# codelion/adaptive-classifier

Hardware: AMD Instinct MI355X
Metric: predict() queries/sec + kNN GB/s vs HBM roofline, 768-d (higher is better)
Workload: dtype f32

## Files before the change

adaptive-classifier_amd/adaptive_classifier/_native.py:

```python
import ctypes
import os
import subprocess

import torch

_HERE = os.path.dirname(os.path.abspath(__file__))
_LIB_PATH = os.environ.get("AC_LIBACAMD_PATH") or os.path.join(_HERE, "libacamd.so")
_CSRC = os.path.join(os.path.dirname(_HERE), "csrc")
_lib = None

c_void_p, c_int, c_int64, c_size_t, c_float, c_uint64 = (
    ctypes.c_void_p, ctypes.c_int, ctypes.c_int64, ctypes.c_size_t, ctypes.c_float, ctypes.c_uint64)


class NativeError(RuntimeError):
    pass


AC_GEMM_F32, AC_GEMM_BF16X3, AC_GEMM_F16X2 = 0, 1, 2
AC_BERT_LAYERED = 1
AC_BERT_PATH_PACKED, AC_BERT_PATH_PADDED, AC_BERT_PATH_PADDED_MASK = 0, 1, 2


def build(force=False):
# ... 31 lines not shown
        "attn_norm_g", "attn_norm_b", "wqkv", "wqkv_b", "wo", "wo_b", "mlp_norm_g", "mlp_norm_b",
        "wi", "wi_b", "wo2", "wo2_b", "zero_bias", "wqkv3", "wo3", "wi3", "wo23")] + [("wi_interleaved32", c_int)]


class ac_wordpiece_vocab(ctypes.Structure):
    _fields_ = [("keys", c_void_p), ("offs", c_void_p), ("ids", c_void_p), ("lens", c_void_p), ("blob", c_void_p),
                ("slots", c_int), ("max_piece_bytes", c_int), ("unk_id", c_int), ("cls_id", c_int), ("sep_id", c_int),
                ("pad_id", c_int), ("lower_case", c_int)]


class ac_bert_weights(ctypes.Structure):
    _fields_ = [(n, c_void_p) for n in (
        "word_emb", "pos_emb", "type_emb", "emb_ln_g", "emb_ln_b",
        "qkv_w", "qkv_b", "ao_w", "ao_b", "ln1_g", "ln1_b",
        "ff1_w", "ff1_b", "ff2_w", "ff2_b", "ln2_g", "ln2_b",
        "qkv_w3", "ao_w3", "ff1_w3", "ff2_w3", "qkv_wh", "ao_wh", "ff1_wh", "ff2_wh")]


_SIGNATURES = {
    "ac_last_error": (ctypes.c_char_p, []),
    "ac_version": (c_int, []),
    "ac_device_info": (c_int, [ctypes.POINTER(c_int), ctypes.POINTER(c_int), ctypes.POINTER(c_size_t)]),
    "ac_device_cus": (c_int, [ctypes.POINTER(c_int), ctypes.POINTER(c_int)]),
    "ac_persistent_launches": (c_int, [ctypes.POINTER(c_int64), ctypes.POINTER(c_int64)]),
    "ac_knn_l2_topk_workspace": (c_int, [c_int64, c_int, c_int, c_int, ctypes.POINTER(c_size_t)]),
    "ac_knn_l2_topk": (c_int, [c_void_p, c_int64, c_int64, c_int, c_void_p, c_int, c_int64, c_int, c_int64,
                               c_void_p, c_void_p, c_void_p, c_size_t, c_void_p, c_void_p]),
    "ac_knn_l2_topk_x": (c_int, [c_void_p, c_int64, c_int64, c_int, c_void_p, c_int, c_int64, c_int, c_int64,
                                 c_void_p, c_void_p, c_void_p, c_void_p, c_size_t, c_void_p, c_void_p]),
    "ac_knn_ip_topk_workspace": (c_int, [c_int64, c_int, c_int, c_int, ctypes.POINTER(c_size_t)]),
    "ac_knn_ip_topk": (c_int, [c_void_p, c_int64, c_int64, c_int, c_void_p, c_int, c_int64, c_int, c_int64,
                               c_void_p, c_void_p, c_void_p, c_size_t, c_void_p, c_void_p]),
    "ac_knn_ip_topk_x": (c_int, [c_void_p, c_int64, c_int64, c_int, c_void_p, c_int, c_int64, c_int, c_int64,
                                 c_void_p, c_void_p, c_void_p, c_void_p, c_size_t, c_void_p, c_void_p]),
    "ac_topk_merge_ip_f64": (c_int, [c_void_p, c_void_p, c_int, c_int, c_int, c_void_p, c_void_p, c_void_p]),
    "ac_knn_store_bytes": (c_int, [c_int64, c_int, ctypes.POINTER(c_size_t), ctypes.POINTER(c_size_t)]),
    "ac_knn_prepare_store": (c_int, [c_void_p, c_int64, c_int64, c_int, c_void_p, c_void_p, c_void_p]),
    "ac_knn_update_store": (c_int, [c_void_p, c_int64, c_int64, c_int64, c_int, c_void_p, c_void_p, c_int64, c_int64, c_void_p, c_void_p]),
    "ac_knn_l2_topk_batch_workspace": (c_int, [c_int64, c_int, c_int, c_int, ctypes.POINTER(c_size_t)]),
    "ac_knn_l2_topk_batch": (c_int, [c_void_p, c_int64, c_int64, c_int, c_void_p, c_void_p, c_void_p, c_int, c_int64, c_int,
                                     c_int64, c_void_p, c_void_p, c_void_p, c_void_p, c_size_t, c_void_p, c_void_p]),
    "ac_knn_ip_topk_batch_workspace": (c_int, [c_int64, c_int, c_int, c_int, ctypes.POINTER(c_size_t)]),
    "ac_knn_ip_topk_batch": (c_int, [c_void_p, c_int64, c_int64, c_int, c_void_p, c_void_p, c_void_p, c_int, c_int64, c_int,
                                     c_int64, c_void_p, c_void_p, c_void_p, c_void_p, c_size_t, c_void_p, c_void_p]),
    "ac_knn_range_workspace": (c_int, [c_int64, c_int, c_int, ctypes.POINTER(c_size_t)]),
    "ac_knn_l2_range_count": (c_int, [c_void_p, c_int64, c_int64, c_int, c_void_p, c_int, c_int64, c_void_p, c_void_p,
                                      c_void_p, c_size_t, c_void_p, c_void_p]),
    "ac_knn_l2_range_fill": (c_int, [c_void_p, c_int64, c_int64, c_int, c_void_p, c_int, c_int64, c_int64, c_void_p, c_int64,
                                     c_void_p, c_void_p, c_void_p, c_void_p, c_size_t, c_void_p, c_void_p]),
    "ac_knn_ip_range_count": (c_int, [c_void_p, c_int64, c_int64, c_int, c_void_p, c_int, c_int64, c_void_p, c_void_p,
                                      c_void_p, c_size_t, c_void_p, c_void_p]),
    "ac_knn_ip_range_fill": (c_int, [c_void_p, c_int64, c_int64, c_int, c_void_p, c_int, c_int64, c_int64, c_void_p, c_int64,
                                     c_void_p, c_void_p, c_void_p, c_void_p, c_size_t, c_void_p, c_void_p]),
    "ac_knn_l2_topk_sel": (c_int, [c_void_p, c_int64, c_int64, c_int, c_void_p, c_int, c_int64, c_int, c_int64, c_void_p, c_int64,
                                   c_void_p, c_void_p, c_void_p, c_void_p, c_size_t, c_void_p, c_void_p]),
    "ac_knn_ip_topk_sel": (c_int, [c_void_p, c_int64, c_int64, c_int, c_void_p, c_int, c_int64, c_int, c_int64, c_void_p, c_int64,
                                   c_void_p, c_void_p, c_void_p, c_void_p, c_size_t, c_void_p, c_void_p]),
    "ac_knn_l2_topk_ids": (c_int, [c_void_p, c_int64, c_int64, c_int, c_void_p, c_int64, c_void_p, c_int, c_int64, c_int, c_int64,
                                   c_void_p, c_void_p, c_void_p, c_void_p]),
    "ac_knn_ip_topk_ids": (c_int, [c_void_p, c_int64, c_int64, c_int, c_void_p, c_int64, c_void_p, c_int, c_int64, c_int, c_int64,
                                   c_void_p, c_void_p, c_void_p, c_void_p]),
    "ac_knn_sel_pack": (c_int, [c_void_p, c_int64, c_void_p, c_void_p]),
    "ac_knn_sel_classes": (c_int, [c_void_p, c_int64, c_void_p, c_int, c_void_p, c_void_p]),
    "ac_knn_set_profile_events": (c_int, [c_void_p, c_void_p]),
    "ac_topk_merge": (c_int, [c_void_p, c_void_p, c_int, c_int, c_int, c_void_p, c_void_p, c_void_p]),
    "ac_topk_merge_f64": (c_int, [c_void_p, c_void_p, c_int, c_int, c_int, c_void_p, c_void_p, c_void_p]),
    "ac_rows_to_class": (c_int, [c_void_p, c_int64, c_void_p, c_int64, c_void_p, c_int, c_void_p, c_void_p]),
    "ac_proto_scores": (c_int, [c_void_p, c_void_p, c_int, c_int, c_void_p, c_void_p]),
    "ac_synth_unit_rows": (c_int, [c_void_p, c_int64, c_int64, c_int, c_uint64, c_int64, c_void_p]),
    "ac_linear_f32": (c_int, [c_void_p, c_int64, c_void_p, c_int64, c_void_p, c_void_p, c_int64, c_void_p,
                              c_int64, c_int, c_int, c_int, c_int, c_void_p]),
    "ac_gemm_f32": (c_int, [c_int, c_int, c_int, c_int, c_int, c_float, c_void_p, c_int64, c_void_p, c_int64,
                            c_float, c_void_p, c_int64, c_void_p]),
    "ac_gemm_set_arith": (c_int, [c_int]),
    "ac_gemm_get_arith": (c_int, []),
    "ac_gemm_set_variant": (c_int, [c_int]),
    "ac_gemm_debug_stamps": (c_int, [c_void_p, c_int64]),
    "ac_gemm_set_pipe_table": (c_int, [ctypes.c_char_p]),
    "ac_gemm_set_pipe_table_f16": (c_int, [ctypes.c_char_p]),
    "ac_gemm_set_krot": (c_int, [c_int]),
    "ac_gemm_set_ln_fusion": (c_int, [c_int]),
    "ac_gemm_ln_fusion_launches": (c_int64, []),
    "ac_gemm_qkv_attn_launches": (c_int64, []),
    "ac_set_persistent_kernels": (c_int, [c_int]),
    "ac_clock_stamp": (c_int, [c_void_p, c_void_p]),
    "ac_gemm_occupancy": (c_int, [c_int, c_int, ctypes.POINTER(c_int)]),
    "ac_split_bf16x3": (c_int, [c_void_p, c_int64, c_int64, c_int, c_void_p, c_void_p]),
    "ac_split_f16x2": (c_int, [c_void_p, c_int64, c_int64, c_int, c_int, c_void_p, c_void_p]),
    "ac_linear_f16x2": (c_int, [c_void_p, c_void_p, c_void_p, c_void_p, c_int64, c_void_p, c_int64, c_void_p, c_int, c_int,
                                c_int, c_int, c_void_p]),
    "ac_linear_bf16x3": (c_int, [c_void_p, c_int64, c_void_p, c_void_p, c_int64, c_void_p, c_void_p, c_void_p,
                                 c_int64, c_void_p, c_int64, c_void_p, c_int, c_int, c_int, c_int, c_void_p]),
    "ac_head_param_count": (c_int64, [ctypes.POINTER(ac_head_dims)]),
    "ac_head_workspace": (c_int, [ctypes.POINTER(ac_head_dims), c_int, ctypes.POINTER(c_size_t)]),
    "ac_head_forward": (c_int, [ctypes.POINTER(ac_head_dims), c_void_p, c_void_p, c_int64, c_int, c_void_p,
                                c_void_p, c_size_t, c_void_p]),
    "ac_head_fwd_bwd_ce": (c_int, [ctypes.POINTER(ac_head_dims), c_void_p, c_void_p, c_int64, c_void_p,
                                   c_void_p, c_void_p, c_float, c_int, c_void_p, c_void_p, c_void_p, c_size_t,
                                   c_void_p]),
    "ac_head_fwd_bwd_loss": (c_int, [ctypes.POINTER(ac_head_dims), c_void_p, c_void_p, c_int64, c_void_p, c_void_p,
                                     c_int64, c_int, c_void_p, c_void_p, c_float, c_int, c_void_p, c_void_p, c_void_p,
                                     c_size_t, c_void_p]),
    "ac_strategic_workspace": (c_int, [ctypes.POINTER(ac_head_dims), c_int, c_int, ctypes.POINTER(c_size_t)]),
    "ac_strategic_best_response": (c_int, [ctypes.POINTER(ac_head_dims), c_void_p, c_void_p, c_int64, c_int, c_void_p,
                                           c_void_p, c_int, c_void_p, c_int, c_int, c_void_p, c_void_p, c_float, c_uint64,
                                           c_void_p, c_void_p, c_void_p, c_void_p, c_int64, c_void_p, c_void_p, c_size_t,
                                           c_void_p]),
    "ac_head_fwd_bwd_strategic": (c_int, [ctypes.POINTER(ac_head_dims), c_void_p, c_void_p, c_int64, c_void_p, c_void_p,
                                          c_void_p, c_float, c_int, c_uint64, c_int, c_float, c_void_p, c_void_p, c_void_p,
                                          c_void_p, c_size_t, c_void_p]),
    "ac_sigmoid": (c_int, [c_void_p, c_int64, c_void_p, c_void_p]),
    "ac_head_train_step": (c_int, [ctypes.POINTER(ac_head_dims), c_void_p, c_void_p, c_void_p, c_void_p, c_void_p,
                                   c_int64, c_void_p, c_void_p, c_int64, c_int, c_void_p, c_int, c_float, c_uint64,
                                   c_void_p, c_void_p,
                                   c_float, c_float, c_float, c_float, c_float, c_float, c_float, c_int, c_void_p,
                                   c_void_p, c_void_p, c_size_t, c_void_p]),
    "ac_head_train_epoch": (c_int, [ctypes.POINTER(ac_head_dims), c_void_p, c_void_p, c_void_p, c_void_p, c_void_p,
                                    c_int64, c_void_p, c_void_p, c_int64, c_int, c_void_p, c_int64, c_int, c_float,
                                    c_uint64, c_void_p, c_void_p,
                                    c_float, c_float, c_float, c_float, c_float, c_float, c_float, c_int, c_void_p,
                                    c_void_p, c_void_p, c_size_t, ctypes.POINTER(c_int), c_void_p]),
    "ac_softmax_rows": (c_int, [c_void_p, c_int, c_int, c_void_p, c_void_p]),
    "ac_l2_normalize_rows": (c_int, [c_void_p, c_int64, c_int, c_int, c_void_p, c_int64, c_void_p]),
    "ac_fisher_accumulate": (c_int, [c_void_p, c_float, c_void_p, c_int64, c_void_p]),
    "ac_ewc_loss": (c_int, [c_void_p, c_void_p, c_void_p, c_int64, c_float, c_void_p, c_void_p, c_void_p]),
    "ac_ewc_adamw_step": (c_int, [c_void_p, c_void_p, c_void_p, c_void_p, c_void_p, c_void_p, c_int64, c_float,
                                  c_float, c_float, c_float, c_float, c_float, c_float, c_int, c_void_p,
                                  c_void_p, c_void_p]),
    "ac_memory_add_prune": (c_int, [c_void_p, c_void_p, c_int, c_int, c_void_p]),
    "ac_blend_topk": (c_int, [c_void_p, c_void_p, c_int, c_void_p, c_int, c_void_p, c_void_p, c_int, c_int, c_int,
                              c_void_p, c_void_p, c_void_p, c_void_p]),
    "ac_modernbert_workspace": (c_int, [ctypes.POINTER(ac_modernbert_config), c_int, c_int, ctypes.POINTER(c_size_t)]),
    "ac_modernbert_encode_cls": (c_int, [ctypes.POINTER(ac_modernbert_config), ctypes.POINTER(ac_modernbert_weights),
                                         c_void_p, c_void_p, c_int, c_int, c_void_p, c_int64, c_void_p, c_size_t,
                                         c_void_p]),
    "ac_modernbert_encode_cls_packed": (c_int, [ctypes.POINTER(ac_modernbert_config), ctypes.POINTER(ac_modernbert_weights),
                                                c_void_p, c_int, c_int, c_void_p, c_void_p, c_int, c_int, c_void_p, c_int64,
                                                c_void_p, c_size_t, c_void_p]),
    "ac_wordpiece_hash": (c_uint64, [c_void_p, c_int, c_int]),
    "ac_wordpiece_encode": (c_int, [c_void_p, c_void_p, c_int, ctypes.POINTER(ac_wordpiece_vocab), c_int, c_void_p, c_void_p,
                                    c_void_p, c_void_p]),
    "ac_bert_workspace": (c_int, [ctypes.POINTER(ac_bert_config), c_int, c_int, ctypes.POINTER(c_size_t)]),
    "ac_bert_pack": (c_int, [c_void_p, c_int, c_int, c_void_p, c_void_p, c_void_p, c_void_p]),
    "ac_bert_encode_cls_packed": (c_int, [ctypes.POINTER(ac_bert_config), ctypes.POINTER(ac_bert_weights), c_void_p, c_void_p,
                                          c_int, c_int, c_void_p, c_void_p, c_int, c_int, c_void_p, c_int64, c_void_p, c_size_t,
                                          c_void_p]),
    "ac_bert_unpad_last_wait_ns": (ctypes.c_longlong, []),
    "ac_predict_post": (c_int, [c_void_p, c_void_p, c_int, c_void_p, c_int64, c_void_p, c_int, c_void_p, c_int, c_int, c_void_p, c_void_p,
                                c_int, c_int, c_int, c_void_p, c_size_t, c_void_p, c_void_p]),
    "ac_host_alloc": (c_int, [c_size_t, ctypes.POINTER(c_void_p)]),
    "ac_host_free": (c_int, [c_void_p]),
    "ac_bert_encode_cls_unpad": (c_int, [ctypes.POINTER(ac_bert_config), ctypes.POINTER(ac_bert_weights), c_void_p, c_void_p,
                                         c_void_p, c_int, c_int, c_void_p, c_int64, c_void_p, c_size_t, c_int,
                                         ctypes.POINTER(c_int), ctypes.POINTER(c_int), c_void_p]),
    "ac_bert_encode_cls_opts": (c_int, [ctypes.POINTER(ac_bert_config), ctypes.POINTER(ac_bert_weights), c_void_p,
                                        c_void_p, c_void_p, c_int, c_int, c_void_p, c_int64, c_void_p, c_size_t, c_int,
                                        ctypes.POINTER(c_int), c_void_p]),
    "ac_bert_one_launch_status": (c_int, [ctypes.POINTER(ac_bert_config), c_int, c_int, c_void_p, c_size_t,
                                          ctypes.POINTER(c_int), c_void_p]),
    "ac_bert_ln_fusion_clear": (c_int, [c_void_p, c_size_t, c_void_p]),
    "ac_bert_ln_fusion_status": (c_int, [ctypes.POINTER(ac_bert_config), c_int, c_int, c_void_p, c_size_t,
                                         ctypes.POINTER(c_int), c_void_p]),
    "ac_bert_encode_cls": (c_int, [ctypes.POINTER(ac_bert_config), ctypes.POINTER(ac_bert_weights), c_void_p,
                                   c_void_p, c_void_p, c_int, c_int, c_void_p, c_int64, c_void_p, c_size_t,
                                   c_void_p]),
}
# ... 54 lines not shown
```

adaptive-classifier_amd/csrc/bert.hip:

```cpp
#include "common.h"
#include "attention_core.h"

#include <math.h>
#include <atomic>
#include <chrono>
#include <string.h>

namespace {

typedef float f32x4 __attribute__((ext_vector_type(4)));
constexpr int kMaxVec = 8;

__device__ __forceinline__ float wave_sum(float v) {
#pragma unroll
    for (int o = 1; o < 64; o <<= 1) v += __shfl_xor(v, o);
    return v;
}

template <bool F16 = false>
__device__ __forceinline__ void layernorm_store(f32x4 (&x)[kMaxVec], int H, int lane, const float* g,
                                                const float* b, float eps, float* dst, uint16_t* planes = nullptr,
                                                int64_t rows = 0, int64_t row = 0) {
    const int nv = H >> 2;
    float s = 0.f;
// ... 575 lines not shown
            ac::linear_f16x2_takes(T, H, I);
    return p;
}
void launch_embed(const ac_bert_config& c, const ac_bert_weights* w, const EncodePlan& pn, const int64_t* d_ids, const int64_t* d_type_ids,
                  int rows, int S, float* x, uint16_t* xp, const int32_t* tok_src, const int32_t* t_dev, hipStream_t stream) {
    const int H = c.hidden, tok_blocks = (rows + 3) / 4;
    if (pn.f16)
        hipLaunchKernelGGL(embed_ln_kernel<true>, dim3(tok_blocks), dim3(256), 0, stream, d_ids, d_type_ids, rows, S, H,
                           w->word_emb, w->pos_emb, w->type_emb, w->emb_ln_g, w->emb_ln_b, c.ln_eps, x, xp, tok_src, t_dev);
    else
        hipLaunchKernelGGL(embed_ln_kernel<false>, dim3(tok_blocks), dim3(256), 0, stream, d_ids, d_type_ids, rows, S, H,
                           w->word_emb, w->pos_emb, w->type_emb, w->emb_ln_g, w->emb_ln_b, c.ln_eps, x,
                           pn.pl ? xp : nullptr, tok_src, t_dev);
}
constexpr int kPreCtl = 1, kPreEmbed = 2;
int bert_encode_impl(const ac_bert_config* cfg, const ac_bert_weights* w, const int64_t* d_ids, const int64_t* d_type_ids,
                     const int64_t* d_mask, int b, int S, const int32_t* cu, const int32_t* tok_src, int T, int Smax,
                     float* d_out, int64_t ldo, void* d_ws, size_t ws_bytes, hipStream_t stream, int pre = 0) {
    int rc;
    const ac_bert_config& c = *cfg;
    const BertWs ws = bert_ws(c, b, S);
    AC_REQUIRE(d_ws && ws_bytes >= ws.total, AC_EWORKSPACE, "bert_encode_cls: workspace %zu < %zu", ws_bytes, ws.total);
    char* base = (char*)d_ws;
    float* x = (float*)(base + ws.x);
    float* qkv = (float*)(base + ws.qkv);
    float* ctx = (float*)(base + ws.ctx);
    float* y = (float*)(base + ws.y);
    float* ffn = (float*)(base + ws.ffn);
    const int H = c.hidden, I = c.intermediate;

    uint16_t* xp = (uint16_t*)(base + ws.xp);
    uint16_t* ctxp = (uint16_t*)(base + ws.ctxp);
    uint16_t* ffnp = (uint16_t*)(base + ws.ffnp);
    const EncodePlan pn = encode_plan(c, w, T);
    const bool wplanes = pn.wplanes, pl = pn.pl;
    const bool f16 = pn.f16;
    const bool fuse_ln = pl && c.layers > 1 && ac::pipe_ln_applies(T, H, H) && ac::pipe_ln_applies(T, H, I);
    unsigned* ln_abort = (unsigned*)base;
    if (!(pre & kPreCtl)) {
        hipLaunchKernelGGL(ln_verdict_roll_kernel, dim3(1), dim3(1), 0, stream, ln_abort);
        AC_LAUNCH_CHECK();
    }
    unsigned* ln_count = (unsigned*)(base + ws.lnctl);
    const int ln_panels = ac::pipe_ln_panels(T);
    if (fuse_ln && !(pre & kPreCtl)) AC_HIP_CHECK(hipMemsetAsync(base + ws.lnctl, 0, ws.lnctl_bytes, stream));

    if (!(pre & kPreEmbed)) {
        launch_embed(c, w, pn, d_ids, d_type_ids, T, S, x, xp, tok_src, nullptr, stream);
        AC_LAUNCH_CHECK();
    }
    const int dh = c.hidden / c.heads;
    const float scale = 1.0f / sqrtf((float)dh);
    const int32_t* cu_at = cu;
    const bool fuse_attn = pl && c.layers > 1 && dh == 64 && (cu || !d_mask) && ac::qkv_attn_applies(T, H, c.heads, Smax);
    if (fuse_attn && !cu) {
        int32_t* cuw = (int32_t*)(base + ws.cu);
        hipLaunchKernelGGL(iota_cu_kernel, dim3((b + 256) / 256), dim3(256), 0, stream, cuw, b, S);
        AC_LAUNCH_CHECK();
        cu_at = cuw;
    }
    int32_t* tile_seq = (int32_t*)(base + ws.tile_seq);
    unsigned* attn_xchg = nullptr;
    if (fuse_attn) {
        if (!(pre & kPreCtl) || !cu) {
            rc = ac::qkv_attn_tile_seq(cu_at, b, T, tile_seq, stream);
            if (rc) return rc;
        }
        if (ac::qkv_attn_exchange_applies(T, c.heads, (int)f16)) {
            attn_xchg = (unsigned*)(base + ws.attn_xchg);
            if (!(pre & kPreCtl)) AC_HIP_CHECK(hipMemsetAsync(attn_xchg, 0, ws.attn_xchg_bytes, stream));
        }
    }
    for (int l = 0; l < c.layers; ++l) {
        const uint16_t* qkv_w3 = wplanes ? w->qkv_w3[l] : nullptr;
        const uint16_t* ao_w3 = wplanes ? w->ao_w3[l] : nullptr;
        const uint16_t* ff1_w3 = wplanes ? w->ff1_w3[l] : nullptr;
        const uint16_t* ff2_w3 = wplanes ? w->ff2_w3[l] : nullptr;
        const bool last = (l == c.layers - 1);
        const int Ml = last ? b : T;
        const bool lp = pl && !last;
        const float* resid = x;
        int64_t ldres = last ? (int64_t)S * H : H;
        const bool q_cls_only = last && T >= 4 * b;
        if (last && cu) {
            hipLaunchKernelGGL(gather_rows_kernel, dim3((b + 3) / 4), dim3(256), 0, stream, x, cu, b, H, ffn);
            AC_LAUNCH_CHECK();
            resid = ffn;
            ldres = H;
        }
        if (fuse_attn && !last) {
            rc = ac::launch_gemm_pipe_qkv_attn(xp, T, f16 ? w->qkv_wh[l] : qkv_w3, 3 * H, w->qkv_b[l], T, H, c.heads, cu_at, tile_seq, b, Smax,
                                               scale, ctxp, qkv, stream, (int)f16, attn_xchg, (unsigned)(l + 1), ln_abort);
            if (rc) return rc;
            const int nbound = (T - 1) / ac::kQkvAttnRows;
            if (nbound > 0 && !attn_xchg) {
                hipLaunchKernelGGL((attention_mfma_kernel<false, 64>), dim3((Smax + 31) / 32, c.heads, nbound), dim3(64), 0, stream, qkv,
                                   nullptr, S, H, scale, ctx, ctxp, nullptr, nullptr, -1, cu_at, (int64_t)T, (int)f16, ac::kQkvAttnRows, b);
                AC_LAUNCH_CHECK();
            }
        } else if (q_cls_only) {
            const int64_t HH = (int64_t)H * H;
            rc = f16 ? ac::linear_f16x2(xp, w->qkv_wh[l] + (int64_t)H * 8, w->qkv_b[l] + H, nullptr, 0, qkv + H, 3 * H, nullptr, T, 2 * H, H, 0,
                                        stream, 3 * H)
                     : ac::linear_f32(x, H, w->qkv_w[l] + HH, H, w->qkv_b[l] + H, nullptr, 0, qkv + H, 3 * H, T, 2 * H, H, 0, nullptr, 1.f,
                                      stream, 0.f, 0, qkv_w3 ? qkv_w3 + (int64_t)H * 8 : nullptr, pl ? xp : nullptr, nullptr, 3 * H);
            if (rc) return rc;
            rc = ac::linear_f32_splitk(resid, ldres, w->qkv_w[l], H, w->qkv_b[l], nullptr, 0, y, H, b, H, H, 0, qkv_w3, ctx,
                                       (size_t)T * H * sizeof(float), stream, 3 * H);
        } else {
            rc = f16 ? ac::linear_f16x2(xp, w->qkv_wh[l], w->qkv_b[l], nullptr, 0, qkv, 3 * H, nullptr, T, 3 * H, H, 0, stream)
                     : ac::linear_f32(x, H, w->qkv_w[l], H, w->qkv_b[l], nullptr, 0, qkv, 3 * H, T, 3 * H, H, 0, nullptr, 1.f,
                                      stream, 0.f, 0, qkv_w3, pl ? xp : nullptr);
        }
        if (rc) return rc;
        if (fuse_attn && !last) {
        } else if (last) {
            const float* qc = q_cls_only ? y : nullptr;
            if (dh == 64 && Smax <= 32)
                hipLaunchKernelGGL((attention_cls_kernel<false, 64, 32>), dim3(c.heads, b), dim3(64), 0, stream, qkv, d_mask, S, H, scale,
                                   ctx, nullptr, nullptr, -1, cu, qc);
            else if (dh == 64)
                hipLaunchKernelGGL((attention_cls_kernel<false, 64>), dim3(c.heads, b), dim3(64), 0, stream, qkv, d_mask, S, H, scale,
                                   ctx, nullptr, nullptr, -1, cu, qc);
            else
                hipLaunchKernelGGL((attention_cls_kernel<false, 32>), dim3(c.heads, b), dim3(64), 0, stream, qkv, d_mask, S, H, scale,
                                   ctx, nullptr, nullptr, -1, cu, qc);
        } else {
            if (dh == 64)
                hipLaunchKernelGGL((attention_mfma_kernel<false, 64>), dim3((Smax + 31) / 32, c.heads, b), dim3(64), 0, stream, qkv,
                                   d_mask, S, H, scale, ctx, lp ? ctxp : nullptr, nullptr, nullptr, -1, cu, (int64_t)T, (int)f16);
            else
                hipLaunchKernelGGL((attention_mfma_kernel<false, 32>), dim3((Smax + 31) / 32, c.heads, b), dim3(64), 0, stream, qkv,
                                   d_mask, S, H, scale, ctx, lp ? ctxp : nullptr, nullptr, nullptr, -1, cu, (int64_t)T, (int)f16);
        }
        AC_LAUNCH_CHECK();
        const int lblocks = (Ml + 3) / 4;
        const bool fl = fuse_ln && lp;
        if (fl) {
            rc = ac::launch_gemm_pipe_ln(ctxp, Ml, f16 ? w->ao_wh[l] : ao_w3, H, w->ao_b[l], x, H, x, H, Ml, H, H, w->ln1_g[l], w->ln1_b[l], c.ln_eps,
                                         base + ws.lnpart, ln_count + (size_t)(2 * l) * ln_panels, ln_abort, xp, stream, (int)f16);
            if (rc) return rc;
        } else {
            rc = last ? ac::linear_f32_splitk(ctx, H, w->ao_w[l], H, w->ao_b[l], resid, ldres, y, H, Ml, H, H, 0, ao_w3, qkv,
                                              (size_t)T * 3 * H * sizeof(float), stream)
                      : (f16 ? ac::linear_f16x2(ctxp, w->ao_wh[l], w->ao_b[l], resid, ldres, y, H, nullptr, Ml, H, H, 0, stream)
                             : ac::linear_f32(ctx, H, w->ao_w[l], H, w->ao_b[l], resid, ldres, y, H, Ml, H, H, 0, nullptr, 1.f, stream,
                                              0.f, 0, ao_w3, lp ? ctxp : nullptr));
            if (rc) return rc;
            launch_ln(f16, lblocks, stream, y, Ml, H, w->ln1_g[l], w->ln1_b[l], c.ln_eps, last ? ctx : x, lp ? xp : nullptr, (int64_t)H);
            AC_LAUNCH_CHECK();
        }
        float* x1 = last ? ctx : x;
        rc = last ? ac::linear_f32_splitk(x1, H, w->ff1_w[l], H, w->ff1_b[l], nullptr, 0, ffn, I, Ml, I, H, 2, ff1_w3, qkv,
                                          (size_t)T * 3 * H * sizeof(float), stream)
                  : (f16 ? ac::linear_f16x2(xp, w->ff1_wh[l], w->ff1_b[l], nullptr, 0, nullptr, I, ffnp, Ml, I, H, 2, stream)
                         : ac::linear_f32(x1, H, w->ff1_w[l], H, w->ff1_b[l], nullptr, 0, ffn, I, Ml, I, H, 2, nullptr, 1.f, stream,
                                          0.f, 0, ff1_w3, lp ? xp : nullptr, lp ? ffnp : nullptr));
        if (rc) return rc;
        if (fl) {
            rc = ac::launch_gemm_pipe_ln(ffnp, Ml, f16 ? w->ff2_wh[l] : ff2_w3, H, w->ff2_b[l], x, H, x, H, Ml, H, I, w->ln2_g[l], w->ln2_b[l], c.ln_eps,
                                         base + ws.lnpart, ln_count + (size_t)(2 * l + 1) * ln_panels, ln_abort, xp, stream, (int)f16);
            if (rc) return rc;
            continue;
        }
        if (last && tail_fused()) {
            int ks = 0;
            rc = ac::linear_f32_splitk(ffn, I, w->ff2_w[l], I, w->ff2_b[l], x1, H, y, H, Ml, H, I, 0, ff2_w3, qkv,
                                       (size_t)T * 3 * H * sizeof(float), stream, 0, &ks);
            if (rc) return rc;
            if (ks > 0) {
                hipLaunchKernelGGL(splitk_ln_normalize_kernel, dim3(b), dim3(64), 0, stream, qkv, ks, b, H, w->ff2_b[l], x1, (int64_t)H,
                                   w->ln2_g[l], w->ln2_b[l], c.ln_eps, d_out, ldo);
                AC_LAUNCH_CHECK();
                return AC_OK;
            }
            launch_ln(f16, lblocks, stream, y, Ml, H, w->ln2_g[l], w->ln2_b[l], c.ln_eps, x, nullptr, (int64_t)H);
            AC_LAUNCH_CHECK();
            break;
        }
        rc = last ? ac::linear_f32_splitk(ffn, I, w->ff2_w[l], I, w->ff2_b[l], x1, H, y, H, Ml, H, I, 0, ff2_w3, qkv,
                                          (size_t)T * 3 * H * sizeof(float), stream)
                  : (f16 ? ac::linear_f16x2(ffnp, w->ff2_wh[l], w->ff2_b[l], x1, H, y, H, nullptr, Ml, H, I, 0, stream)
                         : ac::linear_f32(ffn, I, w->ff2_w[l], I, w->ff2_b[l], x1, H, y, H, Ml, H, I, 0, nullptr, 1.f, stream, 0.f, 0,
                                          ff2_w3, lp ? ffnp : nullptr));
        if (rc) return rc;
        launch_ln(f16, lblocks, stream, y, Ml, H, w->ln2_g[l], w->ln2_b[l], c.ln_eps, x, lp ? xp : nullptr, (int64_t)H);
        AC_LAUNCH_CHECK();
    }
    hipLaunchKernelGGL(cls_normalize_kernel, dim3((b + 3) / 4), dim3(256), 0, stream, x, b, 1, H, d_out, ldo);
    AC_LAUNCH_CHECK();
    return AC_OK;
}

}

extern "C" int ac_bert_encode_cls_opts(const ac_bert_config* cfg, const ac_bert_weights* w, const int64_t* d_ids,
                                       const int64_t* d_type_ids, const int64_t* d_mask, int b, int S,
                                       float* d_out, int64_t ldo, void* d_ws, size_t ws_bytes, int opts, int* used_one_launch,
// ... 339 lines not shown
```

adaptive-classifier_amd/csrc/common.h:

```cpp
#pragma once
#include <atomic>
#include <hip/hip_runtime.h>
#include <stdarg.h>
#include <stdint.h>
#include <stdio.h>

#include "../../include/acamd.h"

namespace ac {

void set_error(const char* fmt, ...);

struct DevInfo {
    int cus;
    int lds_per_block;
    size_t hbm_bytes;
    int hw_cus;
};
const DevInfo& dev_info();

bool test_hooks_enabled();
#define AC_TEST_HOOK_ONLY(name)                                                                                                   \
    do {                                                                                                                          \
        if (!ac::test_hooks_enabled()) {                                                                                          \
            ac::set_error(name ": process-wide switches are test hooks; this process did not enable them (AC_TEST_HOOKS=1)");    \
            return AC_EUNSUPPORTED;                                                                                               \
        }                                                                                                                         \
    } while (0)

bool first_call_on_device(std::atomic<unsigned long long>& done);

#define AC_HIP_CHECK(expr)                                                              \
    do {                                                                                \
        hipError_t _e = (expr);                                                         \
        if (_e != hipSuccess) {                                                         \
            ac::set_error("%s failed: %s (%s:%d)", #expr, hipGetErrorString(_e),        \
                          __FILE__, __LINE__);                                          \
            return AC_EHIP;                                                             \
        }                                                                               \
    } while (0)

#define AC_REQUIRE(cond, code, ...)                                                     \
    do {                                                                                \
        if (!(cond)) {                                                                  \
            ac::set_error(__VA_ARGS__);                                                 \
            return (code);                                                              \
        }                                                                               \
    } while (0)

#define AC_LAUNCH_CHECK()                                                               \
    do {                                                                                \
        hipError_t _e = hipGetLastError();                                              \
        if (_e != hipSuccess) {                                                         \
            ac::set_error("kernel launch failed: %s (%s:%d)", hipGetErrorString(_e),    \
                          __FILE__, __LINE__);                                          \
            return AC_EHIP;                                                             \
        }                                                                               \
    } while (0)

__host__ __device__ static inline size_t align_up(size_t x, size_t a) { return (x + a - 1) / a * a; }
static inline int next_pow2(int x) { int p = 1; while (p < x) p <<= 1; return p; }

int linear_f32(const float* A, int64_t lda, const float* W, int64_t ldw, const float* bias,
               const float* residual, int64_t ldr, float* C, int64_t ldc, int M, int N, int K, int act,
               const uint8_t* mask, float mask_scale, hipStream_t stream, float drop_p = 0.f,
               uint64_t drop_seed = 0, const uint16_t* W_planes = nullptr, const uint16_t* A_planes = nullptr,
               uint16_t* C_planes = nullptr, int64_t w_plane_rows = 0);
int linear_f32_splitk(const float* A, int64_t lda, const float* W, int64_t ldw, const float* bias, const float* residual,
                      int64_t ldr, float* C, int64_t ldc, int M, int N, int K, int act, const uint16_t* W_planes, float* scratch,
                      size_t scratch_bytes, hipStream_t stream, int64_t w_plane_rows = 0, int* partials_only = nullptr);
bool pipe_ln_applies(int M, int N, int K);
size_t pipe_ln_part_bytes(int M, int N);
int pipe_ln_panels(int M);
int launch_gemm_pipe_ln(const uint16_t* Ap, int64_t a_rows, const uint16_t* Wp, int64_t w_rows, const float* bias,
                        const float* residual, int64_t ldr, float* C, int64_t ldc, int M, int N, int K, const float* gamma,
                        const float* beta, float eps, void* part, unsigned* count, unsigned* abort_flag, uint16_t* planes,
                        hipStream_t stream, int f16 = 0);
constexpr int kQkvAttnRows = 256;
constexpr int kQkvAttnCu = 264;
bool qkv_attn_applies(int M, int H, int heads, int smax);
size_t qkv_attn_tile_seq_bytes(int M);
int qkv_attn_tile_seq(const int32_t* cu, int b, int M, int32_t* tile_seq, hipStream_t stream);
bool qkv_attn_exchange_applies(int M, int heads, int f16);
int launch_gemm_pipe_qkv_attn(const uint16_t* Ap, int64_t a_rows, const uint16_t* Wp, int64_t w_rows, const float* bias, int M, int H,
                              int heads, const int32_t* cu, const int32_t* tile_seq, int b, int smax, float scale, uint16_t* ctx_planes,
                              float* qkv, hipStream_t stream, int f16 = 0, unsigned* exchange = nullptr, unsigned epoch = 0,
                              unsigned* abort_flag = nullptr);
bool linear_takes_planes(int M, int N, int K);

__host__ __device__ static inline bool dropout_keep(uint64_t seed, uint64_t idx, float p) {
    uint64_t z = seed + idx * 0x9E3779B97F4A7C15ull;
    z = (z ^ (z >> 30)) * 0xBF58476D1CE4E5B9ull;
    z = (z ^ (z >> 27)) * 0x94D049BB133111EBull;
    z ^= z >> 31;
    return (float)(z >> 40) * (1.0f / 16777216.0f) >= p;
}
#ifdef __HIPCC__
typedef __bf16 bf16x2_t __attribute__((ext_vector_type(2)));
typedef float f32x2_t __attribute__((ext_vector_type(2)));
typedef float f32x4_t __attribute__((ext_vector_type(4)));

__device__ __forceinline__ uint32_t pack_bf16(float a, float b) {
    const f32x2_t f = {a, b};
    return __builtin_bit_cast(uint32_t, __builtin_convertvector(f, bf16x2_t));
}
__device__ __forceinline__ void split2(float a, float b, uint32_t& h, uint32_t& m, uint32_t& l) {
    h = pack_bf16(a, b);
    const float ra = a - __uint_as_float(h << 16), rb = b - __uint_as_float(h & 0xffff0000u);
    m = pack_bf16(ra, rb);
    const float sa = ra - __uint_as_float(m << 16), sb = rb - __uint_as_float(m & 0xffff0000u);
    l = pack_bf16(sa, sb);
}
__device__ __forceinline__ void split4(const f32x4_t& x, uint2& H, uint2& M, uint2& L) {
    split2(x[0], x[1], H.x, M.x, L.x);
    split2(x[2], x[3], H.y, M.y, L.y);
}
__device__ __forceinline__ void split8(const f32x4_t& x0, const f32x4_t& x1, uint4& H, uint4& M, uint4& L) {
    split2(x0[0], x0[1], H.x, M.x, L.x);
    split2(x0[2], x0[3], H.y, M.y, L.y);
    split2(x1[0], x1[1], H.z, M.z, L.z);
    split2(x1[2], x1[3], H.w, M.w, L.w);
}
constexpr int kF16ActLog2 = 6, kF16WLog2 = 10;
constexpr float kF16ActScale = (float)(1 << kF16ActLog2), kF16OutScale = 1.0f / (float)(1 << (kF16ActLog2 + kF16WLog2));
typedef _Float16 f16x2_t __attribute__((ext_vector_type(2)));
__device__ __forceinline__ void split2h(float a, float b, float s, uint32_t& h, uint32_t& l) {
    a *= s; b *= s;
    const f16x2_t hv = {(_Float16)a, (_Float16)b};
    const f16x2_t lv = {(_Float16)(a - (float)hv[0]), (_Float16)(b - (float)hv[1])};
    h = __builtin_bit_cast(uint32_t, hv);
    l = __builtin_bit_cast(uint32_t, lv);
}
__device__ __forceinline__ void split4h(const f32x4_t& x, float s, uint2& H, uint2& L) {
    split2h(x[0], x[1], s, H.x, L.x);
    split2h(x[2], x[3], s, H.y, L.y);
}
__device__ __forceinline__ void split8h(const f32x4_t& x0, const f32x4_t& x1, float s, uint4& H, uint4& L) {
    split2h(x0[0], x0[1], s, H.x, L.x);
    split2h(x0[2], x0[3], s, H.y, L.y);
    split2h(x1[0], x1[1], s, H.z, L.z);
    split2h(x1[2], x1[3], s, H.w, L.w);
}
__device__ __forceinline__ void emit_planes4(uint16_t* p, int64_t plane, const f32x4_t& v, int f16) {
    if (f16) {
        uint2 H, L;
        split4h(v, kF16ActScale, H, L);
        *reinterpret_cast<uint2*>(p) = H;
        *reinterpret_cast<uint2*>(p + plane) = L;
    } else {
        uint2 H, M, L;
        split4(v, H, M, L);
        *reinterpret_cast<uint2*>(p) = H;
        *reinterpret_cast<uint2*>(p + plane) = M;
        *reinterpret_cast<uint2*>(p + 2 * plane) = L;
    }
}
__device__ __forceinline__ void emit_planes8(uint16_t* p, int64_t plane, const f32x4_t& v0, const f32x4_t& v1, int f16) {
    if (f16) {
        uint4 H, L;
        split8h(v0, v1, kF16ActScale, H, L);
        *reinterpret_cast<uint4*>(p) = H;
        *reinterpret_cast<uint4*>(p + plane) = L;
    } else {
        uint4 H, M, L;
        split8(v0, v1, H, M, L);
        *reinterpret_cast<uint4*>(p) = H;
        *reinterpret_cast<uint4*>(p + plane) = M;
        *reinterpret_cast<uint4*>(p + 2 * plane) = L;
    }
}
__device__ __forceinline__ float gelu_erf(float x) {
// ... 166 lines not shown
```

include/acamd.h:

```cpp
#ifndef ACAMD_H
#define ACAMD_H

#include <stddef.h>
#include <stdint.h>

#ifdef __cplusplus
extern "C" {
#endif

#define AC_OK            0
#define AC_EINVAL       -1
#define AC_EUNSUPPORTED -2
#define AC_EWORKSPACE   -3
#define AC_EHIP         -4

typedef void* ac_stream_t;

const char* ac_last_error(void);
int ac_version(void);
int ac_device_info(int* cu_count, int* lds_bytes_per_block, size_t* hbm_bytes);
int ac_device_cus(int* chip_cus, int* active_cus);
int ac_persistent_launches(int64_t* head_epoch, int64_t* bert_small);


// ... 70 lines not shown
                          const float* d_radius, int64_t* d_lims,
                          void* d_ws, size_t ws_bytes, int32_t* d_stats,
                          ac_stream_t stream);
int ac_knn_ip_range_fill(const float* d_P, int64_t N, int64_t ldP, int D,
                         const float* d_Q, int nq, int64_t ldQ,
                         int64_t row_offset, const int64_t* d_lims, int64_t capacity,
                         float* d_outD, double* d_outD64, int64_t* d_outI,
                         void* d_ws, size_t ws_bytes, int32_t* d_stats,
                         ac_stream_t stream);

int ac_knn_l2_topk_sel(const float* d_P, int64_t N, int64_t ldP, int D,
                       const float* d_Q, int nq, int64_t ldQ, int k,
                       int64_t row_offset, const uint64_t* d_sel, int64_t sel_bit0,
                       float* d_outD, double* d_outD64, int64_t* d_outI,
                       void* d_ws, size_t ws_bytes, int32_t* d_stats,
                       ac_stream_t stream);
int ac_knn_ip_topk_sel(const float* d_P, int64_t N, int64_t ldP, int D,
                       const float* d_Q, int nq, int64_t ldQ, int k,
                       int64_t row_offset, const uint64_t* d_sel, int64_t sel_bit0,
                       float* d_outD, double* d_outD64, int64_t* d_outI,
                       void* d_ws, size_t ws_bytes, int32_t* d_stats,
                       ac_stream_t stream);
int ac_knn_l2_topk_ids(const float* d_P, int64_t N, int64_t ldP, int D,
                       const int64_t* d_ids, int64_t M,
                       const float* d_Q, int nq, int64_t ldQ, int k,
                       int64_t row_offset,
                       float* d_outD, double* d_outD64, int64_t* d_outI,
                       ac_stream_t stream);
int ac_knn_ip_topk_ids(const float* d_P, int64_t N, int64_t ldP, int D,
                       const int64_t* d_ids, int64_t M,
                       const float* d_Q, int nq, int64_t ldQ, int k,
                       int64_t row_offset,
                       float* d_outD, double* d_outD64, int64_t* d_outI,
                       ac_stream_t stream);
int ac_knn_sel_pack(const uint8_t* d_mask, int64_t n, uint64_t* d_sel, ac_stream_t stream);
int ac_knn_sel_classes(const int32_t* d_row_class, int64_t n, const uint8_t* d_class_on, int n_classes,
                       uint64_t* d_sel, ac_stream_t stream);

int ac_knn_set_profile_events(void* start_event, void* stop_event);

int ac_topk_merge(const float* d_D_in, const int64_t* d_I_in, int shards,
                  int nq, int k, float* d_outD, int64_t* d_outI,
                  ac_stream_t stream);
int ac_topk_merge_f64(const double* d_D_in, const int64_t* d_I_in, int shards,
                      int nq, int k, float* d_outD, int64_t* d_outI,
                      ac_stream_t stream);
int ac_topk_merge_ip_f64(const double* d_D_in, const int64_t* d_I_in, int shards,
                         int nq, int k, float* d_outD, int64_t* d_outI,
                         ac_stream_t stream);

int ac_proto_scores(const float* d_D, const int64_t* d_I, int nq, int k,
                    float* d_out, ac_stream_t stream);

int ac_rows_to_class(const int64_t* d_I, int64_t n, const int32_t* d_row_class,
                     int64_t nrows, const int64_t* d_class_lut, int nlut,
                     int64_t* d_out, ac_stream_t stream);

int ac_synth_unit_rows(float* d_out, int64_t n, int64_t ld, int D,
                       uint64_t seed, int64_t row_offset, ac_stream_t stream);


int ac_linear_f32(const float* d_A, int64_t lda, const float* d_W, int64_t ldw,
                  const float* d_bias, const float* d_residual, int64_t ldr,
                  float* d_C, int64_t ldc, int M, int N, int K, int act,
                  ac_stream_t stream);

int ac_gemm_f32(int transA, int transB, int M, int N, int K, float alpha,
                const float* d_A, int64_t lda, const float* d_B, int64_t ldb,
                float beta, float* d_C, int64_t ldc, ac_stream_t stream);

#define AC_GEMM_F32 0
#define AC_GEMM_BF16X3 1
#define AC_GEMM_F16X2 2
int ac_gemm_set_arith(int mode);
int ac_gemm_get_arith(void);
int ac_gemm_set_variant(int variant);
int ac_gemm_debug_stamps(unsigned long long* d_buf, int64_t capacity_workgroups);
int ac_gemm_set_pipe_table(const char* spec);
int ac_gemm_set_krot(int on);
int ac_gemm_set_pipe_table_f16(const char* spec);
int ac_gemm_set_ln_fusion(int on);
int64_t ac_gemm_ln_fusion_launches(void);
int64_t ac_gemm_qkv_attn_launches(void);

int ac_set_persistent_kernels(int mask);

int ac_clock_stamp(unsigned long long* d_out16, ac_stream_t stream);

int ac_gemm_occupancy(int kernel, int tm, int* blocks_per_cu);

int ac_split_bf16x3(const float* d_X, int64_t ldx, int64_t rows, int K,
                    uint16_t* d_planes, ac_stream_t stream);

int ac_split_f16x2(const float* d_X, int64_t ldx, int64_t rows, int K, int scale_log2,
                   uint16_t* d_planes, ac_stream_t stream);

int ac_linear_f16x2(const uint16_t* d_A_planes, const uint16_t* d_W_planes, const float* d_bias,
                    const float* d_residual, int64_t ldr, float* d_C, int64_t ldc, uint16_t* d_C_planes,
                    int M, int N, int K, int act, ac_stream_t stream);

int ac_linear_bf16x3(const float* d_A, int64_t lda, const uint16_t* d_A_planes,
                     const float* d_W, int64_t ldw, const uint16_t* d_W_planes,
                     const float* d_bias, const float* d_residual, int64_t ldr,
                     float* d_C, int64_t ldc, uint16_t* d_C_planes,
                     int M, int N, int K, int act, ac_stream_t stream);

typedef struct {
    int D, H1, H2, C;
} ac_head_dims;

int64_t ac_head_param_count(const ac_head_dims* dims);

int ac_head_workspace(const ac_head_dims* dims, int B, size_t* bytes);

int ac_head_forward(const ac_head_dims* dims, const float* d_params,
                    const float* d_X, int64_t ldx, int B, float* d_logits,
                    void* d_ws, size_t ws_bytes, ac_stream_t stream);

int ac_head_fwd_bwd_ce(const ac_head_dims* dims, const float* d_params,
                       const float* d_X, int64_t ldx, const int64_t* d_y,
                       const uint8_t* d_mask1, const uint8_t* d_mask2,
                       float dropout_p, int B, float* d_loss, float* d_grads,
                       void* d_ws, size_t ws_bytes, ac_stream_t stream);

#define AC_REDUCE_SCRATCH_BYTES 8192

#define AC_LOSS_CE          0
#define AC_LOSS_BCE_SIGMOID 1
#define AC_LOSS_CE_SIGMOID  2
#define AC_LOSS_STEPWISE 0x100

int ac_head_fwd_bwd_loss(const ac_head_dims* dims, const float* d_params,
                         const float* d_X, int64_t ldx, const int64_t* d_y,
                         const float* d_targets, int64_t ldt, int loss_kind,
                         const uint8_t* d_mask1, const uint8_t* d_mask2,
                         float dropout_p, int B, float* d_loss, float* d_grads,
                         void* d_ws, size_t ws_bytes, ac_stream_t stream);

int ac_sigmoid(const float* d_in, int64_t n, float* d_out, ac_stream_t stream);

int ac_head_train_step(const ac_head_dims* dims, float* d_params, float* d_m,
                       float* d_v, float* d_grads, const float* d_X, int64_t ldx,
                       const int64_t* d_y, const float* d_targets, int64_t ldt,
                       int loss_kind, const int64_t* d_index, int B,
                       float dropout_p, uint64_t dropout_seed,
                       const float* d_fisher, const float* d_old,
                       float lambda_over_B, float max_grad_norm, float lr,
                       float beta1, float beta2, float eps, float weight_decay,
                       int step, float* d_out, float* d_loss_accum,
                       void* d_ws, size_t ws_bytes, ac_stream_t stream);

int ac_head_train_epoch(const ac_head_dims* dims, float* d_params, float* d_m,
                        float* d_v, float* d_grads, const float* d_X, int64_t ldx,
                        const int64_t* d_y, const float* d_targets, int64_t ldt,
                        int loss_kind, const int64_t* d_order, int64_t n_total, int batch,
                        float dropout_p, uint64_t seed0,
                        const float* d_fisher, const float* d_old, float lambda_B,
                        float max_grad_norm, float lr, float beta1, float beta2,
                        float eps, float weight_decay, int step0,
                        float* d_out, float* d_loss_accum,
                        void* d_ws, size_t ws_bytes, int* steps_done, ac_stream_t stream);

#define AC_STRAT_COST_SEPARABLE 0
#define AC_STRAT_COST_LINEAR    1
#define AC_STRAT_MASK_NONE      0
#define AC_STRAT_MASK_EXPLICIT  1
// ... 211 lines not shown
```

Measured before the change: 51610.

## Fold CLS-only last-layer attention through K/V weights to skip K/V projection

In the last BERT layer, when only CLS queries are needed, this skips the K/V projection GEMM over all T tokens. It folds the CLS query through Wk (g = q·Wk per head), scores keys directly against the hidden states x with an online softmax, forms a softmax-weighted sum of x, and then projects through Wv. The goal is to replace a T×2H×H GEMM with work proportional to b·heads·H. The cost is three new kernels, different numerics (the K bias is dropped, which is fine because softmax does not change under a constant shift), and a gate based on head dims and size limits.

```diff
diff --git a/adaptive-classifier_amd/adaptive_classifier/_native.py b/adaptive-classifier_amd/adaptive_classifier/_native.py
--- a/adaptive-classifier_amd/adaptive_classifier/_native.py
+++ b/adaptive-classifier_amd/adaptive_classifier/_native.py
@@ -137,6 +137,7 @@
     "ac_gemm_set_ln_fusion": (c_int, [c_int]),
     "ac_gemm_ln_fusion_launches": (c_int64, []),
     "ac_gemm_qkv_attn_launches": (c_int64, []),
+    "ac_bert_cls_fold_launches": (c_int64, []),
     "ac_set_persistent_kernels": (c_int, [c_int]),
     "ac_clock_stamp": (c_int, [c_void_p, c_void_p]),
     "ac_gemm_occupancy": (c_int, [c_int, c_int, ctypes.POINTER(c_int)]),
diff --git a/adaptive-classifier_amd/csrc/bert.hip b/adaptive-classifier_amd/csrc/bert.hip
--- a/adaptive-classifier_amd/csrc/bert.hip
+++ b/adaptive-classifier_amd/csrc/bert.hip
@@ -681,6 +681,7 @@
         const float* resid = x;
         int64_t ldres = last ? (int64_t)S * H : H;
         const bool q_cls_only = last && T >= 4 * b;
+        const bool cls_fold = q_cls_only && ac::cls_fold_applies(b, T, H, c.heads);
         if (last && cu) {
             hipLaunchKernelGGL(gather_rows_kernel, dim3((b + 3) / 4), dim3(256), 0, stream, x, cu, b, H, ffn);
             AC_LAUNCH_CHECK();
@@ -699,7 +700,7 @@
             }
         } else if (q_cls_only) {
             const int64_t HH = (int64_t)H * H;
-            rc = f16 ? ac::linear_f16x2(xp, w->qkv_wh[l] + (int64_t)H * 8, w->qkv_b[l] + H, nullptr, 0, qkv + H, 3 * H, nullptr, T, 2 * H, H, 0,
+            rc = cls_fold ? AC_OK : f16 ? ac::linear_f16x2(xp, w->qkv_wh[l] + (int64_t)H * 8, w->qkv_b[l] + H, nullptr, 0, qkv + H, 3 * H, nullptr, T, 2 * H, H, 0,
                                         stream, 3 * H)
                      : ac::linear_f32(x, H, w->qkv_w[l] + HH, H, w->qkv_b[l] + H, nullptr, 0, qkv + H, 3 * H, T, 2 * H, H, 0, nullptr, 1.f,
                                       stream, 0.f, 0, qkv_w3 ? qkv_w3 + (int64_t)H * 8 : nullptr, pl ? xp : nullptr, nullptr, 3 * H);
@@ -713,6 +714,10 @@
         }
         if (rc) return rc;
         if (fuse_attn && !last) {
+        } else if (cls_fold) {
+            rc = ac::cls_fold_attention(x, y, w->qkv_w[l], w->qkv_b[l], d_mask, cu, b, S, H, c.heads, scale, qkv, ctx + (size_t)b * H, ctx,
+                                        stream);
+            if (rc) return rc;
         } else if (last) {
             const float* qc = q_cls_only ? y : nullptr;
             if (dh == 64 && Smax <= 32)
diff --git a/adaptive-classifier_amd/csrc/cls_fold.hip b/adaptive-classifier_amd/csrc/cls_fold.hip
--- /dev/null
+++ b/adaptive-classifier_amd/csrc/cls_fold.hip
@@ -0,0 +1,257 @@
+#include "common.h"
+#include "gemm_common.h"
+#include "grid_sync.h"
+
+#include <math.h>
+#include <stdlib.h>
+
+namespace {
+
+using acg::f32x4;
+using acg::f32x16;
+using acg::acc_row32;
+
+constexpr int kSuThreads = 1024;
+constexpr int kSuKeys = 64;
+constexpr int kSuMaxHg = 16;
+constexpr int kSuMaxVec = 8;
+constexpr size_t kSuGBytes = 48 * 1024;
+
+template <int DHT>
+__global__ __launch_bounds__(256) void cls_fold_g_kernel(const float* __restrict__ q, const float* __restrict__ Wk, int b, int H,
+                                                         int heads, float* __restrict__ g) {
+    constexpr int KH = DHT / 2;
+    const int lane = threadIdx.x & 63, wave = threadIdx.x >> 6;
+    const int nt = blockIdx.x * 4 + wave;
+    if (nt * 32 >= H) return;
+    const int head = blockIdx.y, s0 = blockIdx.z * 32;
+    const int i = lane & 31, hh = lane >> 5;
+    int srow = s0 + i; if (srow > b - 1) srow = b - 1;
+    const float* qp = q + (int64_t)srow * H + head * DHT + hh * KH;
+    const float* wp = Wk + (int64_t)(head * DHT + hh * KH) * H + nt * 32 + i;
+    f32x4 a[KH / 4];
+    float w[KH];
+#pragma unroll
+    for (int e = 0; e < KH / 4; ++e) a[e] = *reinterpret_cast<const f32x4*>(qp + 4 * e);
+#pragma unroll
+    for (int t = 0; t < KH; ++t) w[t] = wp[(int64_t)t * H];
+    f32x16 acc;
+#pragma unroll
+    for (int r = 0; r < 16; ++r) acc[r] = 0.f;
+#pragma unroll
+    for (int t = 0; t < KH; ++t) acc = __builtin_amdgcn_mfma_f32_32x32x2f32(a[t >> 2][t & 3], w[t], acc, 0, 0, 0);
+#pragma unroll
+    for (int r = 0; r < 16; ++r) {
+        const int row = s0 + acc_row32(r, lane);
+        if (row < b) g[((int64_t)row * heads + head) * H + nt * 32 + i] = acc[r];
+    }
+}
+
+__global__ __launch_bounds__(kSuThreads) void cls_fold_su_kernel(const float* __restrict__ x, const int64_t* __restrict__ mask,
+                                                                 const int32_t* __restrict__ cu, int S_, int H, int heads, int hg,
+                                                                 float scale, float* gu, float* __restrict__ nonempty) {
+    extern __shared__ __attribute__((aligned(16))) float gs[];
+    __shared__ __attribute__((aligned(16))) float sc[kSuKeys][kSuMaxHg];
+    __shared__ __attribute__((aligned(16))) float corr_s[kSuMaxHg];
+    __shared__ float l_s[kSuMaxHg];
+    const int tid = threadIdx.x, lane = tid & 63, wave = tid >> 6;
+    const int s = blockIdx.y, h0 = blockIdx.x * hg;
+    const int nh = (heads - h0) < hg ? (heads - h0) : hg;
+    const int nv = H >> 2;
+    const int64_t row0 = cu ? (int64_t)cu[s] : (int64_t)s * S_;
+    const int S = cu ? cu[s + 1] - cu[s] : S_;
+    float* gus = gu + ((int64_t)s * heads + h0) * H;
+    for (int i = tid; i < nh * nv; i += kSuThreads) reinterpret_cast<f32x4*>(gs)[i] = reinterpret_cast<const f32x4*>(gus)[i];
+    for (int i = tid; i < kSuKeys * kSuMaxHg; i += kSuThreads) (&sc[0][0])[i] = 0.f;
+    if (tid < kSuMaxHg) corr_s[tid] = 1.f;
+    const int c4 = tid % nv, hs = tid / nv;
+    const bool active = 4 * hs < nh;
+    f32x4 acc[4];
+#pragma unroll
+    for (int i = 0; i < 4; ++i) acc[i] = f32x4{0.f, 0.f, 0.f, 0.f};
+    float m = -INFINITY, l = 0.f;
+    const float* xs = x + row0 * H;
+    for (int k0 = 0; k0 < S; k0 += kSuKeys) {
+        const int nk = (S - k0) < kSuKeys ? (S - k0) : kSuKeys;
+        __syncthreads();
+        for (int t = wave; t < kSuKeys; t += kSuThreads / 64) {
+            const bool valid = t < nk && (!mask || mask[(int64_t)s * S_ + k0 + t] != 0);
+            if (!valid) {
+                if (lane < nh) sc[t][lane] = -INFINITY;
+                continue;
+            }
+            const f32x4* xr = reinterpret_cast<const f32x4*>(xs + (int64_t)(k0 + t) * H);
+            f32x4 xv[kSuMaxVec];
+#pragma unroll
+            for (int e = 0; e < kSuMaxVec; ++e) {
+                const int c = lane + 64 * e;
+                xv[e] = c < nv ? xr[c] : f32x4{0.f, 0.f, 0.f, 0.f};
+            }
+            for (int h = 0; h < nh; ++h) {
+                const f32x4* gr = reinterpret_cast<const f32x4*>(gs) + h * nv;
+                float d = 0.f;
+#pragma unroll
+                for (int e = 0; e < kSuMaxVec; ++e) {
+                    const int c = lane + 64 * e;
+                    if (c < nv) {
+                        const f32x4 gv = gr[c];
+                        d = fmaf(xv[e].x, gv.x, d); d = fmaf(xv[e].y, gv.y, d); d = fmaf(xv[e].z, gv.z, d); d = fmaf(xv[e].w, gv.w, d);
+                    }
+                }
+                d = acp::wave_sum(d);
+                if (lane == 0) sc[t][h] = d * scale;
+            }
+        }
+        __syncthreads();
+        if (wave < nh) {
+            const float v = sc[lane][wave];
+            float cmax = v;
+#pragma unroll
+            for (int off = 1; off < 64; off <<= 1) cmax = fmaxf(cmax, __shfl_xor(cmax, off));
+            const float m_new = fmaxf(m, cmax);
+            float p = 0.f, corr = 1.f;
+            if (m_new != -INFINITY) {
+                corr = expf(m - m_new);
+                p = expf(v - m_new);
+            }
+            sc[lane][wave] = p;
+            l = l * corr + acp::wave_sum(p);
+            m = m_new;
+            if (lane == 0) corr_s[wave] = corr;
+        }
+        __syncthreads();
+        if (active) {
+            const f32x4 cr = *reinterpret_cast<const f32x4*>(&corr_s[4 * hs]);
+#pragma unroll
+            for (int i = 0; i < 4; ++i) acc[i] *= cr[i];
+            const f32x4* xc = reinterpret_cast<const f32x4*>(xs + (int64_t)k0 * H) + c4;
+#pragma unroll 4
+            for (int t = 0; t < nk; ++t) {
+                const f32x4 xv = xc[(int64_t)t * nv];
+                const f32x4 p = *reinterpret_cast<const f32x4*>(&sc[t][4 * hs]);
+#pragma unroll
+                for (int i = 0; i < 4; ++i) {
+                    acc[i].x = fmaf(p[i], xv.x, acc[i].x); acc[i].y = fmaf(p[i], xv.y, acc[i].y);
+                    acc[i].z = fmaf(p[i], xv.z, acc[i].z); acc[i].w = fmaf(p[i], xv.w, acc[i].w);
+                }
+            }
+        }
+    }
+    if (wave < nh && lane == 0) l_s[wave] = l;
+    __syncthreads();
+    if (active) {
+#pragma unroll
+        for (int i = 0; i < 4; ++i) {
+            const int h = 4 * hs + i;
+            if (h < nh) {
+                const float lv = l_s[h];
+                f32x4 o = {0.f, 0.f, 0.f, 0.f};
+                if (lv > 0.f) { o.x = acc[i].x / lv; o.y = acc[i].y / lv; o.z = acc[i].z / lv; o.w = acc[i].w / lv; }
+                reinterpret_cast<f32x4*>(gus)[h * nv + c4] = o;
+            }
+        }
+    }
+    if (tid < nh) nonempty[(int64_t)s * heads + h0 + tid] = l_s[tid] > 0.f ? 1.f : 0.f;
+}
+
+constexpr int kCtxWaves = 8;
+__global__ __launch_bounds__(kCtxWaves * 64) void cls_fold_ctx_kernel(const float* __restrict__ u, const float* __restrict__ nonempty,
+                                                                      const float* __restrict__ Wv, const float* __restrict__ bv, int b,
+                                                                      int H, int heads, int dh, float* __restrict__ ctx) {
+    __shared__ float red[kCtxWaves][16][64];
+    const int tid = threadIdx.x, lane = tid & 63, wave = tid >> 6;
+    const int head = blockIdx.y, s0 = blockIdx.z * 32, j0 = head * dh + blockIdx.x * 32;
+    const int i = lane & 31, h = lane >> 5;
+    int arow = s0 + i; if (arow > b - 1) arow = b - 1;
+    const float* ap = u + ((int64_t)arow * heads + head) * H + 8 * h;
+    const float* wp = Wv + (int64_t)(j0 + i) * H + 8 * h;
+    const int K = H;
+    f32x16 acc;
+#pragma unroll
+    for (int r = 0; r < 16; ++r) acc[r] = 0.f;
+    const f32x4 zero = {0.f, 0.f, 0.f, 0.f};
+    auto load = [&](int s, f32x4 (&a)[2], f32x4 (&w)[2]) {
+        const int k = 16 * (kCtxWaves * s + wave);
+        if (k + 8 * h < K) {
+            a[0] = *reinterpret_cast<const f32x4*>(ap + k); a[1] = *reinterpret_cast<const f32x4*>(ap + k + 4);
+            w[0] = *reinterpret_cast<const f32x4*>(wp + k); w[1] = *reinterpret_cast<const f32x4*>(wp + k + 4);
+        } else {
+            a[0] = a[1] = w[0] = w[1] = zero;
+        }
+    };
+    const int nslots = (K + 16 * kCtxWaves - 1) / (16 * kCtxWaves);
+    f32x4 a0[2], w0[2], a1[2], w1[2];
+    load(0, a0, w0);
+    for (int s = 0; s < nslots; s += 2) {
+        load(s + 1, a1, w1);
+#pragma unroll
+        for (int e = 0; e < 2; ++e)
+#pragma unroll
+            for (int c = 0; c < 4; ++c) acc = __builtin_amdgcn_mfma_f32_32x32x2f32(a0[e][c], w0[e][c], acc, 0, 0, 0);
+        load(s + 2, a0, w0);
+#pragma unroll
+        for (int e = 0; e < 2; ++e)
+#pragma unroll
+            for (int c = 0; c < 4; ++c) acc = __builtin_amdgcn_mfma_f32_32x32x2f32(a1[e][c], w1[e][c], acc, 0, 0, 0);
+    }
+#pragma unroll
+    for (int r = 0; r < 16; ++r) red[wave][r][lane] = acc[r];
+    __syncthreads();
+#pragma unroll
+    for (int e = 0; e < 2; ++e) {
+        const int o = tid + 512 * e;
+        const int r = o >> 6, l = o & 63;
+        const float v = (((red[0][r][l] + red[1][r][l]) + (red[2][r][l] + red[3][r][l])) +
+                         ((red[4][r][l] + red[5][r][l]) + (red[6][r][l] + red[7][r][l])));
+        const int row = s0 + acc_row32(r, l);
+        const int col = j0 + (l & 31);
+        if (row < b) ctx[(int64_t)row * H + col] = nonempty[(int64_t)row * heads + head] != 0.f ? v + bv[col] : 0.f;
+    }
+}
+
+int su_heads_per_group(int H, int heads) {
+    for (int ng = 1; ng <= heads; ++ng) {
+        const int hg = (heads + ng - 1) / ng;
+        if ((size_t)hg * H * sizeof(float) <= kSuGBytes && hg <= kSuMaxHg && (H / 4) * ((hg + 3) / 4) <= kSuThreads) return hg;
+    }
+    return 0;
+}
+
+std::atomic<long long> g_cls_fold_launches{0};
+
+}
+
+namespace ac {
+
+bool cls_fold_applies(int b, int64_t T, int H, int heads) {
+    if (const char* e = getenv("AC_BERT_CLS_FOLD")) { if (atoi(e) == 0) return false; }
+    const int dh = H / heads;
+    return b > 0 && (dh == 64 || dh == 32) && dh * heads == H && H <= 64 * 4 * kSuMaxVec && su_heads_per_group(H, heads) > 0 &&
+           (int64_t)b * heads * H <= T * 3 * H;
+}
+
+int cls_fold_attention(const float* x, const float* q_cls, const float* w_qkv, const float* b_qkv, const int64_t* mask, const int32_t* cu,
+                       int b, int S, int H, int heads, float scale, float* gu, float* nonempty, float* ctx, hipStream_t stream) {
+    const int dh = H / heads, hg = su_heads_per_group(H, heads);
+    AC_REQUIRE(hg > 0 && (dh == 64 || dh == 32), AC_EUNSUPPORTED, "cls_fold: H=%d heads=%d unsupported", H, heads);
+    const float* Wk = w_qkv + (int64_t)H * H;
+    const float* Wv = w_qkv + 2 * (int64_t)H * H;
+    const dim3 ggrid((H / 32 + 3) / 4, heads, (b + 31) / 32);
+    if (dh == 64)
+        hipLaunchKernelGGL((cls_fold_g_kernel<64>), ggrid, dim3(256), 0, stream, q_cls, Wk, b, H, heads, gu);
+    else
+        hipLaunchKernelGGL((cls_fold_g_kernel<32>), ggrid, dim3(256), 0, stream, q_cls, Wk, b, H, heads, gu);
+    AC_LAUNCH_CHECK();
+    hipLaunchKernelGGL(cls_fold_su_kernel, dim3((heads + hg - 1) / hg, b), dim3(kSuThreads), (size_t)hg * H * sizeof(float), stream, x, mask,
+                       cu, S, H, heads, hg, scale, gu, nonempty);
+    AC_LAUNCH_CHECK();
+    hipLaunchKernelGGL(cls_fold_ctx_kernel, dim3(dh / 32, heads, (b + 31) / 32), dim3(kCtxWaves * 64), 0, stream, gu, nonempty, Wv,
+                       b_qkv + 2 * H, b, H, heads, dh, ctx);
+    AC_LAUNCH_CHECK();
+    g_cls_fold_launches.fetch_add(1, std::memory_order_relaxed);
+    return AC_OK;
+}
+
+}
+
+extern "C" int64_t ac_bert_cls_fold_launches(void) { return (int64_t)g_cls_fold_launches.load(std::memory_order_relaxed); }
diff --git a/adaptive-classifier_amd/csrc/common.h b/adaptive-classifier_amd/csrc/common.h
--- a/adaptive-classifier_amd/csrc/common.h
+++ b/adaptive-classifier_amd/csrc/common.h
@@ -87,6 +87,9 @@
                               float* qkv, hipStream_t stream, int f16 = 0, unsigned* exchange = nullptr, unsigned epoch = 0,
                               unsigned* abort_flag = nullptr);
 bool linear_takes_planes(int M, int N, int K);
+bool cls_fold_applies(int b, int64_t T, int H, int heads);
+int cls_fold_attention(const float* x, const float* q_cls, const float* w_qkv, const float* b_qkv, const int64_t* mask, const int32_t* cu,
+                       int b, int S, int H, int heads, float scale, float* gu, float* nonempty, float* ctx, hipStream_t stream);
 
 __host__ __device__ static inline bool dropout_keep(uint64_t seed, uint64_t idx, float p) {
     uint64_t z = seed + idx * 0x9E3779B97F4A7C15ull;
diff --git a/include/acamd.h b/include/acamd.h
--- a/include/acamd.h
+++ b/include/acamd.h
@@ -176,6 +176,7 @@
 int ac_gemm_set_ln_fusion(int on);
 int64_t ac_gemm_ln_fusion_launches(void);
 int64_t ac_gemm_qkv_attn_launches(void);
+int64_t ac_bert_cls_fold_launches(void);
 
 int ac_set_persistent_kernels(int mask);
 
```

New measurement: 51690 (median of 2 runs). No clear change (+0.2%).
